# dcmlr/groundgrid

Hardware: AMD Instinct MI355X
Metric: point clouds/s (Velodyne-64, ~120k pts, 120m/0.33m grid) (higher is better)
Workload: dtype f32+f64 (the reference's mixed float/double arithmetic, bit-exact)

## Files before the change

groundgrid_amd/csrc/gg_context.hip:

```cpp
#include <float.h>
#include <math.h>
#include <stdio.h>
#include <string.h>

#include <algorithm>
#include <atomic>
#include <condition_variable>
#include <cstdlib>
#include <cstdio>
#include <functional>
#include <mutex>
#include <string>
#include <thread>
#include <vector>
#include <chrono>

#include <dlfcn.h>
#include <sched.h>
#include <unistd.h>

#include "gg_internal.h"
#include "host_helper.h"
#include "scroll_core.h"
#include "sweep_core.h"
// ... 1045 lines not shown
    g.tiles_c = (n + TILE - 1) / TILE;
    g.T = g.tiles_r * g.tiles_c;
    g.resolution = res;
    g.inv_resolution = 1.0 / res;
    g.length0 = g.length1 = (double)n * res;
    g.half0 = 0.5 * g.length0;
    g.half1 = 0.5 * g.length1;
    g.resolution_f = (float)res;
    g.min_dist_squared = geom.min_dist_squared;
    g.center = n / 2 - 1;
    a.hist_pitch = (g.T + 3) & ~3;
    a.n_slots = n_slots;
    if (g.T > 65535 || (size_t)4 * a.hist_pitch * sizeof(uint32_t) > 150 * 1024) {
        gg_destroy(ctx);
        return GG_ERR_GEOMETRY;
    }
    a.PW = g.T <= 1024 ? (n_slots >= PW_BIG_CONTEXT_SLOTS ? 2048 : 1024) : 8192;
    if (getenv("GG_PW")) a.PW = atoi(getenv("GG_PW"));
    if (a.PW < 64 || a.PW % 64 != 0) {
        gg_destroy(ctx);
        return GG_ERR_INVALID;
    }
    a.tune_sweep_waves = getenv("GG_SWEEP_WAVES") ? atoi(getenv("GG_SWEEP_WAVES")) : 0;
    a.tune_sweep_gpw = getenv("GG_SWEEP_GPW") ? atoi(getenv("GG_SWEEP_GPW")) : 0;
    a.tune_sweep_split = getenv("GG_SWEEP_SPLIT") ? atoi(getenv("GG_SWEEP_SPLIT")) : 0;
    a.tune_sweep_pair = getenv("GG_SWEEP_PAIR") ? atoi(getenv("GG_SWEEP_PAIR")) : 0;
    a.tune_sweep_pair_wgs = getenv("GG_SWEEP_PAIR_WGS") ? atoi(getenv("GG_SWEEP_PAIR_WGS")) : 0;
    a.tune_sweep_pair_waves = getenv("GG_SWEEP_PAIR_WAVES") ? atoi(getenv("GG_SWEEP_PAIR_WAVES")) : 0;
    a.tune_front = getenv("GG_FRONT") ? atoi(getenv("GG_FRONT")) : 0;
    a.tune_k2_per_cloud = getenv("GG_K2_PER_CLOUD") ? atoi(getenv("GG_K2_PER_CLOUD")) : 0;
    a.tune_k2_dense_share = getenv("GG_K2_DENSE_SHARE") ? atoi(getenv("GG_K2_DENSE_SHARE")) : 0;
    a.k2_skip = getenv("GG_K2_SKIP") ? atoi(getenv("GG_K2_SKIP")) : 0;
    a.NCH = (int)((max_points + a.PW - 1) / a.PW);
    make_dev_config(ctx->cfg, a.cfg);

    ctx->h_expected.resize((size_t)g.C);
    for (size_t i = 0; i < cellCount; ++i)
        for (size_t j = 0; j < cellCount; ++j) {
            const float dist = (float)hypot((double)i - (double)cellCount / 2.0, (double)j - (double)cellCount / 2.0);
            ctx->h_expected[i + j * cellCount] = atanf(1 / dist) / geom.vertical_point_ang_dist;
        }

    ctx->sweep_params = gg::sweep::make_params(n, res, geom.min_dist_squared, ctx->cfg.occupied_cells_decrease_factor);
    if (gg::sweep_lds_bytes(ctx->sweep_params) > 158 * 1024) {
        gg_destroy(ctx);
        return GG_ERR_GEOMETRY;
    }
    std::vector<uint16_t> tile_rank(g.T), rank_tile(g.T);
    {
        std::vector<std::pair<uint32_t, int>> order(g.T);
        for (int tc = 0; tc < g.tiles_c; ++tc)
            for (int tr = 0; tr < g.tiles_r; ++tr) order[tr + tc * g.tiles_r] = {morton2((uint32_t)tr, (uint32_t)tc), tr + tc * g.tiles_r};
        std::sort(order.begin(), order.end());
        for (int r = 0; r < g.T; ++r) {
            rank_tile[r] = (uint16_t)order[r].second;
            tile_rank[order[r].second] = (uint16_t)r;
        }
    }

    const size_t A = 256;
    size_t off = 0;
    auto carve = [&](size_t bytes) {
        const size_t o = off;
        off = align_up(off + bytes, A);
        return o;
    };
    const size_t C = (size_t)g.C;
    const size_t Cpad = align_up(C * 4, A) / 4;
    const size_t Npad = align_up(max_points * 8, A) / 8;
    const size_t o_expected = carve(C * 4);
    const size_t o_ptable = carve(C * 16);
    const size_t o_trank = carve((size_t)g.T * 2);
    const size_t o_rtile = carve((size_t)g.T * 2);
    const size_t o_rcell0 = carve((size_t)g.T * 4);
    const size_t percall_slot_floats = align_up((size_t)g.T * PERCALL_BLOCK * 4, A) / 4;
    const size_t o_layers = carve((size_t)n_slots * percall_slot_floats * 4);
    a.gpl = make_gp_layout(n);
    a.gp_bits_off = (int)align_up((size_t)a.gpl.elems, 16);
    a.gp_bits_words = (a.gpl.elems / 64 + 2 + 1) & ~1;
    a.gp2_stride = align_up(((size_t)a.gp_bits_off + (size_t)a.gp_bits_words) * 8, A) / 8;
    a.gp_bits_stride = a.gp2_stride;
    const size_t o_gp2 = carve((size_t)n_slots * a.gp2_stride * 8);
    const size_t o_rec = carve((size_t)n_slots * Npad * 8);
    const size_t o_sorted = carve((size_t)n_slots * Npad * 8);
    a.zcell_stride = align_up((Npad + (size_t)32 * g.T + 64) * 4, A) / 4;
    const size_t o_zcell = carve((size_t)n_slots * a.zcell_stride * 4);
    a.hist_stride = align_up((size_t)a.NCH * a.hist_pitch * 4, A) / 4;
    const size_t o_hist = carve((size_t)n_slots * a.hist_stride * 4);
    a.emit_stride = align_up((size_t)a.NCH * 4 * 4, A) / 4;
    const size_t o_emit = carve((size_t)n_slots * a.emit_stride * 4);
    const size_t o_totals = carve((size_t)n_slots * 4 * 4);
    a.tile_start_stride = align_up((size_t)(g.T + 1) * 4, A) / 4;
    const size_t o_tstart = carve((size_t)n_slots * a.tile_start_stride * 4);
    a.tile_live_stride = align_up((size_t)g.T, A);
    const size_t o_tlive = carve((size_t)n_slots * a.tile_live_stride * 4);
    a.tile_list_stride = align_up((size_t)g.T * 16, A) / 16;
    const size_t o_tlist = carve((size_t)n_slots * a.tile_list_stride * 16);
    const size_t o_tlcnt = carve((size_t)n_slots * 2 * 4);
    const size_t o_fsync = carve(((size_t)2 * n_slots + 16) * 4);
    const size_t o_ssync = carve(64);
    const size_t o_fsync2 = carve(((size_t)2 * n_slots + 16) * 4);
    const size_t o_ssync2 = carve(64);
    const size_t o_scansync = carve((size_t)n_slots * SCAN_SYNC_WORDS * 8);
    const size_t o_scansync2 = carve((size_t)n_slots * SCAN_SYNC_WORDS * 8);
    a.sweep_xchg_stride = align_up(std::max<size_t>(gg::sweep_xchg_entries(ctx->sweep_params), 1) * 16, A) / 8;
    const size_t o_xchg = carve((size_t)n_slots * a.sweep_xchg_stride * 8);
    a.sweep_rec_stride = gg::sweep_pair_rec_floats(ctx->sweep_params);
    a.sweep_rec_clouds = a.sweep_rec_stride ? std::min(n_slots, SWEEP_PAIR_MAX_CLOUDS) : 0;
    const size_t o_srec = carve(std::max<size_t>((size_t)a.sweep_rec_clouds * a.sweep_rec_stride * 4, 64));
    const size_t o_params = carve((size_t)PARAM_RING * n_slots * sizeof(CloudParams));
    const size_t o_gparams = carve(sizeof(CloudParams));
    const size_t o_spts = carve(max_points * sizeof(gg_point16));
    const size_t o_slab = carve(max_points);
    const size_t o_sidx = carve(max_points * 4);
    const size_t o_scnt = carve(64);
    const size_t o_scls = carve(max_points);
    const size_t o_scell = carve(max_points * 4);
    size_t o_apts[GG_ASYNC_DEPTH], o_alab[GG_ASYNC_DEPTH], o_aidx[GG_ASYNC_DEPTH], o_acnt[GG_ASYNC_DEPTH];
    for (int k = 0; k < GG_ASYNC_DEPTH; ++k) {
        o_apts[k] = carve(max_points * sizeof(gg_point16));
        o_acnt[k] = carve(64 + max_points * 5 + 64);
// ... 5 lines not shown
    const size_t gp_valid_words = ((size_t)a.gpl.elems + 31) / 32;
    const size_t o_gpvalid = carve(gp_valid_words * 4);
    std::vector<int> gp_border;
    for (int col = 0; col < n; ++col)
        for (int row = 0; row < n; ++row)
            if (std::max(std::abs(row - a.gpl.c), std::abs(col - a.gpl.c)) >= a.gpl.c) gp_border.push_back(gp_index(a.gpl, row, col));
    a.gp_border_n = (int)gp_border.size();
    const size_t o_gpborder = carve(std::max<size_t>(gp_border.size() * 4, 64));
    a.gp_fresh_cell = 1 + (a.gpl.VS - 1) * 64;
    const size_t o_dbg = carve(64 * 8);
    const size_t o_pdbg = carve(2048 * 8);
    const bool k2_timing = getenv("GG_K2_DEBUG") && (atoi(getenv("GG_K2_DEBUG")) == 9 || atoi(getenv("GG_K2_DEBUG")) == 5 || atoi(getenv("GG_K2_DEBUG")) == 6);
    const size_t o_k2dbg = carve(k2_timing ? (size_t)K2_DBG_WGS * 32 * 8 : 64);
    const size_t o_slotmaps = carve((size_t)n_slots * sizeof(ExportMap));
    ctx->arena_bytes = off;
    CREATE_CHK(hipMalloc(&ctx->d_arena, ctx->arena_bytes));
    char *base = (char *)ctx->d_arena;
    CREATE_CHK(hipMemsetAsync(base, 0, ctx->arena_bytes, ctx->stream));

    a.expected = (const float *)(base + o_expected);
    a.patch_table = (const float4 *)(base + o_ptable);
    a.tile_rank = (const uint16_t *)(base + o_trank);
    a.rank_tile = (const uint16_t *)(base + o_rtile);
    a.rank_cell0 = (const uint32_t *)(base + o_rcell0);
    a.layers = (float *)(base + o_layers);
    a.gp2 = (float2 *)(base + o_gp2);
    a.gp_bits = (unsigned long long *)(base + o_gp2) + a.gp_bits_off;
    a.slot_layer_stride = percall_slot_floats;
    a.rec = (uint2 *)(base + o_rec);
    a.sorted = (uint2 *)(base + o_sorted);
    a.zcell = (float *)(base + o_zcell);
    a.point_stride = Npad;
    a.hist = (uint32_t *)(base + o_hist);
    a.chunk_emit = (uint32_t *)(base + o_emit);
    a.totals = (uint32_t *)(base + o_totals);
    a.tile_start = (uint32_t *)(base + o_tstart);
    a.tile_live = (uint32_t *)(base + o_tlive);
    a.tile_list = (uint4 *)(base + o_tlist);
    a.tile_list_cnt = (uint32_t *)(base + o_tlcnt);
    a.front_sync = (uint32_t *)(base + o_fsync);
    a.sweep_sync = (uint32_t *)(base + o_ssync);
    a.front_sync2 = (uint32_t *)(base + o_fsync2);
    a.sweep_sync2 = (uint32_t *)(base + o_ssync2);
    a.scan_sync = (unsigned long long *)(base + o_scansync);
    a.scan_sync2 = (unsigned long long *)(base + o_scansync2);
    {
        const uint32_t first_epoch[4] = {0u, 0u, 1u, 0u};
        CREATE_CHK(hipMemcpyAsync(a.sweep_sync, first_epoch, sizeof first_epoch, hipMemcpyHostToDevice, ctx->stream));
        const uint32_t first_epoch2[4] = {0u, 0u, 0x80000001u, 0u};
        CREATE_CHK(hipMemcpyAsync(a.sweep_sync2, first_epoch2, sizeof first_epoch2, hipMemcpyHostToDevice, ctx->stream));
        CREATE_CHK(hipStreamSynchronize(ctx->stream));
    }
    {
        CREATE_CHK(hipHostMalloc((void **)&ctx->h_dev_error, 64, hipHostMallocMapped));
        *ctx->h_dev_error = 0u;
        void *dptr = nullptr;
        CREATE_CHK(hipHostGetDevicePointer(&dptr, (void *)ctx->h_dev_error, 0));
        a.dev_error = (uint32_t *)dptr;
    }
    a.sweep_xchg = (unsigned long long *)(base + o_xchg);
    a.sweep_rec = a.sweep_rec_clouds ? (float *)(base + o_srec) : nullptr;
    a.pair_dbg = getenv("GG_PAIR_TIMING") ? (unsigned long long *)(base + o_pdbg) : nullptr;
    a.flags = 0;
    a.k2_debug = getenv("GG_K2_DEBUG") ? atoi(getenv("GG_K2_DEBUG")) : 0;
    a.k2_dbg = (unsigned long long *)(base + o_k2dbg);
    a.k3_debug = getenv("GG_K3_DEBUG") ? atoi(getenv("GG_K3_DEBUG")) : 0;
// ... 1801 lines not shown
    hp[0] = CloudParams{};
    hp[0].slot = slot;
    hp[0].n_points = (int)n;
    hp[0].ox = origin[0], hp[0].oy = origin[1], hp[0].oz = origin[2];
    hp[0].pos_x = ctx->pos_x[slot];
    hp[0].pos_y = ctx->pos_y[slot];
    hp[0].no_confidence = ctx->no_confidence[slot] ? 1 : 0;
    hp[0].fresh = 0;
    HIPCHK(ctx, hipMemcpyAsync(dp, hp, sizeof(CloudParams), hipMemcpyHostToDevice, s));
    BatchIO io{};
    io.d_points = ctx->d_stage_pts;
    io.cloud_stride = ctx->max_points;
    io.point_format = GG_POINT16;
    const int front = launch_classify(a, dp, io, 1, (int)n, s);
    if (front == FRONT_THREE_LAUNCHES) launch_scan(a, dp, 1, s);
    if (front != FRONT_ONE_LAUNCH) launch_scatter(a, dp, 1, (int)n, s);
    launch_stage_insert(a, dp, s);
    launch_fill_bytes((uint8_t *)(a.tile_live + (size_t)slot * a.tile_live_stride), (size_t)a.g.T * 4, 0xFF, s);
    launch_decode_classes(a, slot, n, ctx->d_stage_class, ctx->d_stage_cell, s);
    HIPCHK(ctx, hipGetLastError());
    if (out_class) HIPCHK(ctx, hipMemcpyAsync(out_class, ctx->d_stage_class, n, hipMemcpyDeviceToHost, s));
    if (out_cell) HIPCHK(ctx, hipMemcpyAsync(out_cell, ctx->d_stage_cell, n * 4, hipMemcpyDeviceToHost, s));
    HIPCHK(ctx, ctx->ring.recorded(r, s));
    ctx->lazy_pending[slot] = 0;
    if (const int rc = own_stream_mutated_map(ctx)) return rc;
    SYNCCHK(ctx, hipStreamSynchronize(s));
    return GG_OK;
}

extern "C" int gg_debug_set_tuning(gg_context *ctx, const char *key, int value)
{
    if (!ctx || !key || value < 0) return GG_ERR_INVALID;
    if (!strcmp(key, "pw")) return ctx->arena.PW;
    if (!strcmp(key, "graph_replays")) return (int)std::min<long>(ctx->graph_replays, 1 << 30);
    if (!strcmp(key, "fresh_count")) {
        int c = 0;
        for (int k = 0; k < ctx->n_slots; ++k) c += ctx->fresh[k] ? 1 : 0;
        return c;
    }
    if (!strcmp(key, "lazy_count")) {
        int c = 0;
        for (int k = 0; k < ctx->n_slots; ++k) c += ctx->lazy_pending[k] ? 1 : 0;
        return c;
    }
    if (!strcmp(key, "export_variant_default")) return EXPORT_VARIANT_DEFAULT;
    if (!strcmp(key, "import_variant_default")) return IMPORT_VARIANT_DEFAULT;
    if (!strcmp(key, "images_variant_default")) return IMAGES_VARIANT_DEFAULT;
    if (!strcmp(key, "graphs")) {
        ctx->graphs_enabled = value != 0;
        drop_graphs(ctx);
        return GG_OK;
    }
    drop_graphs(ctx);
    if (!strcmp(key, "sweep_waves")) ctx->arena.tune_sweep_waves = value;
    else if (!strcmp(key, "sweep_gpw")) ctx->arena.tune_sweep_gpw = value;
    else if (!strcmp(key, "sweep_split")) ctx->arena.tune_sweep_split = value;
    else if (!strcmp(key, "sweep_pair")) ctx->arena.tune_sweep_pair = value;
    else if (!strcmp(key, "sweep_pair_wgs")) ctx->arena.tune_sweep_pair_wgs = value;
    else if (!strcmp(key, "sweep_pair_waves")) ctx->arena.tune_sweep_pair_waves = value;
    else if (!strcmp(key, "fresh_maps")) ctx->fresh_enabled = value != 0;
    else if (!strcmp(key, "front")) ctx->arena.tune_front = std::min(value, 3);
    else if (!strcmp(key, "sweep_poll_cap")) ctx->arena.tune_sweep_poll_cap = value;
    else if (!strcmp(key, "scan_parts")) ctx->arena.tune_scan_parts = value;
    else if (!strcmp(key, "scan_poll_cap")) ctx->arena.tune_scan_poll_cap = value;
    else if (!strcmp(key, "upload_pieces")) ctx->upload_pieces = value;
    else if (!strcmp(key, "results_direct")) ctx->results_direct = value;
// ... 85 lines not shown
```

groundgrid_amd/csrc/gg_internal.h:

```cpp
#pragma once

#include <hip/hip_runtime.h>
#include <stdint.h>

#include <atomic>
#include <mutex>

#include "groundgrid_hip.h"
#include "gp_layout.h"

namespace gg {

constexpr int TILE = 16;
constexpr int TILE_CELLS = TILE * TILE;
constexpr uint32_t KEY_OUTSIDE = 0xFFFFFFFFu;
constexpr int K2_DBG_WGS = 32768;
constexpr int PW_BIG_CONTEXT_SLOTS = 128;
constexpr int SWEEP_LATENCY_MAX_CLOUDS = 256;
constexpr int K2_MIN_GROUPS_PER_CLOUD = 64;
constexpr int PACKED_TILE_COUNTERS_MIN_T = 1024;
constexpr int K2_LIGHT_MAX = 512;
constexpr int KEY_TILE_SHIFT = 12;
constexpr int SCAN_MAX_PARTS = 16, SCAN_SYNC_WORDS = 1 + SCAN_MAX_PARTS;
constexpr uint32_t KEY_EMIT_BIT = 1u << 10;
// ... 36 lines not shown
    int slot;
    int n_points;
    float ox, oy, oz;
    float base_z;
    double pos_x, pos_y;
    int has_tf;
    int fresh;
    int no_confidence;
    double tf[12];
    int label_shift;
    int io_index;
    int cfg_index = -1;
};

struct Arena {
    Geometry g;
    DevConfig cfg;
    const float *expected;
    const float4 *patch_table;
    const uint16_t *tile_rank;
    const uint16_t *rank_tile;
    const uint32_t *rank_cell0;
    float *layers;  size_t slot_layer_stride;
    const uint32_t *gp_valid;
    float2 *gp2;    size_t gp2_stride;    GpLayout gpl;
    unsigned long long *gp_bits;  size_t gp_bits_stride;  int gp_fresh_cell;
    int gp_bits_off, gp_bits_words;
    const int *gp_border;  int gp_border_n;
    int fresh_launch;
    uint2 *rec;     uint2 *sorted;  size_t point_stride;
    float *zcell;   size_t zcell_stride;
    uint32_t *hist;        size_t hist_stride;
    int hist_pitch;
    uint32_t *front_sync;
    uint32_t *dev_error;
    uint32_t *chunk_emit;  size_t emit_stride;
    uint32_t *totals;
    uint32_t *tile_start;  size_t tile_start_stride;
    uint32_t *tile_live;   size_t tile_live_stride;
    uint4 *tile_list;      size_t tile_list_stride;
    uint32_t *tile_list_cnt;
    unsigned long long *scan_sync;
    uint32_t *front_sync2, *sweep_sync2;
    unsigned long long *scan_sync2;
    uint32_t *sweep_sync;
    unsigned long long *sweep_xchg; size_t sweep_xchg_stride;
    float *sweep_rec; size_t sweep_rec_stride; int sweep_rec_clouds;
    unsigned long long *pair_dbg;
    int n_slots;
    int PW;
    int NCH;
    int tune_sweep_waves;
    int tune_sweep_gpw;
    int tune_sweep_split;
    int tune_sweep_pair;
    int tune_sweep_pair_wgs;
    int tune_sweep_pair_waves;
    int tune_sweep_poll_cap;
    int tune_sweep_fault;
    int tune_scan_fault;
    int tune_scan_poll_cap;
    int tune_scan_parts;
    int tune_front;
    int tune_k2_per_cloud;
    int tune_k2_dense_share;
    int k2_skip;
// ... 251 lines not shown
```

groundgrid_amd/csrc/k1_classify.hip:

```cpp
#include "gg_device.h"
#include "sort_core.h"

#include <algorithm>

namespace gg {

constexpr int WALK_MAX_STEP = 1 << 16;
constexpr int WALK_PACKED_MAX = 12;

struct PointIn {
    float x, y, z;
    int ring;
};

template <int FMT>
GG_DEV PointIn load_point(const void *base, size_t idx)
{
    PointIn p;
    if (FMT == GG_POINT16) {
        const uint4 v = reinterpret_cast<const uint4 *>(base)[idx];
        p.x = __uint_as_float(v.x);
        p.y = __uint_as_float(v.y);
        p.z = __uint_as_float(v.z);
        p.ring = (int)(v.w & 0xFFFFu);
// ... 175 lines not shown
                const uint32_t x = (home + k) % nc, size = q + (x < r ? 1u : 0u);
                const uint32_t t = __hip_atomic_fetch_add(&tickets[x], 1u, __ATOMIC_RELAXED, __HIP_MEMORY_SCOPE_AGENT);
                if (t < size) got = x * q + (x < r ? x : r) + t;
            }
            s_word = got;
        }
        __syncthreads();
        item = s_word;
        if (item == 0xFFFFFFFFu) return;
    } else {
        item = xcd_contiguous_item(blockIdx.x + blockIdx.y * gridDim.x, n_items);
    }
    const int cloud = (int)(item / gridDim.x), bx = (int)(item % gridDim.x);
    const CloudParams &cp = params[cloud];
    DevConfig own_cfg;
    if (SC) load_cloud_config(a, cp.cfg_index, own_cfg);
    const DevConfig &cfg = SC ? own_cfg : a.cfg;
    const int chunk = bx * 4 + wave;
    const int n = cp.n_points;
    const int nch = (n + a.PW - 1) / a.PW;
    const int groups_of_cloud = max(1, (nch + 3) / 4);
    if (bx >= groups_of_cloud) return;
    for (int t = threadIdx.x; t < T; t += 256) lds_tile_rank[t] = a.tile_rank[t];
    uint32_t *hist = lds_hist + wave * words;
    for (int t = lane; t < words; t += 64) hist[t] = 0u;
    __syncthreads();
    const bool active = chunk < nch;

    const float2 *gp2 = gp2_ptr(a, cp.slot);
    const char *pts = reinterpret_cast<const char *>(io.d_points) +
                      (size_t)cp.io_index * io.cloud_stride * (FMT == GG_POINT16 ? 16 : 32);
    uint2 *rec = a.rec + (size_t)cp.slot * a.point_stride;
    const __amdgpu_buffer_rsrc_t ghist = words_rsrc(a.hist + (size_t)cp.slot * a.hist_stride, a.hist_stride);
    const uint32_t row = (uint32_t)chunk * (uint32_t)TP;

    const int base = chunk * a.PW;
    const int end = min(base + a.PW, n);
    if (active) {
        uint32_t n_kept = 0, n_ign = 0, n_outl = 0, n_inmap = 0;
        constexpr int ITEMS = 4;
        PointIn pt[ITEMS];
#pragma unroll
        for (int j = 0; j < ITEMS; ++j) pt[j] = load_point<FMT>(pts, (size_t)min(base + j * 64 + lane, end - 1));
        for (int p0 = base; p0 < end; p0 += 64 * ITEMS) {
            PointIn pt_next[ITEMS];
#pragma unroll
            for (int j = 0; j < ITEMS; ++j) pt_next[j] = load_point<FMT>(pts, (size_t)min(p0 + 64 * ITEMS + j * 64 + lane, end - 1));
            bool valid[ITEMS];
#pragma unroll
            for (int j = 0; j < ITEMS; ++j) valid[j] = p0 + j * 64 + lane < end;
            if (cp.has_tf) {
#pragma unroll
                for (int j = 0; j < ITEMS; ++j) transform_point(cp.tf, pt[j].x, pt[j].y, pt[j].z);
            }
            int gi0[ITEMS], gi1[ITEMS];
            bool inmap_[ITEMS];
            float og[ITEMS];
#pragma unroll
            for (int j = 0; j < ITEMS; ++j) inmap_[j] = locate_point(a, cp, pt[j], gi0[j], gi1[j]) && valid[j];
            const bool need_ground = !cp.no_confidence;
#pragma unroll
            for (int j = 0; j < ITEMS; ++j) og[j] = gp2[(inmap_[j] && need_ground) ? gp_idx(a, gi0[j], gi1[j]) : 0].x;
#pragma unroll
            for (int j = 0; j < ITEMS; ++j) {
                const int p = p0 + j * 64 + lane;
                int cls = GG_CLASS_KEPT;
                bool walk = false;
                if (inmap_[j]) cls = classify_point(a, cfg, cp, pt[j], og[j], walk);
                const int n_walk = __popcll(__ballot(walk));
                if (n_walk > WALK_PACKED_MAX) {
                    if (walk && ray_walk_hits_lane(a, cfg, cp, gp2, pt[j].x, pt[j].y, pt[j].z)) cls = GG_CLASS_OUTLIER;
                } else if (n_walk > 0) {
                    const unsigned long long hits = walk_packed(a, cfg, cp, gp2, pt[j].x, pt[j].y, pt[j].z, walk, lane);
                    if ((hits >> lane) & 1ull) cls = GG_CLASS_OUTLIER;
                }
                uint32_t key = KEY_OUTSIDE;
                if (inmap_[j]) key = make_key(a, lds_tile_rank, gi0[j], gi1[j], cls);
                if (valid[j]) rec[p] = make_uint2(__float_as_uint(pt[j].z), key);
                const bool inmap = key != KEY_OUTSIDE;
                const uint32_t tr = key >> KEY_TILE_SHIFT;
                const LaneRun run = lane_run(inmap ? tr : 0x100000u, lane);
                if (inmap && run.head) {
                    const uint32_t len = (uint32_t)__popcll(run.mask);
                    if (packed)
                        atomicAdd(&hist[tr >> 1], len << ((tr & 1u) * 16u));
                    else
                        atomicAdd(&hist[tr], len);
                }
                const bool emit = inmap && (key & KEY_EMIT_BIT);
                n_inmap += (uint32_t)__popcll(__ballot(inmap));
                n_kept += (uint32_t)__popcll(__ballot(emit && cls == GG_CLASS_KEPT));
                n_ign += (uint32_t)__popcll(__ballot(emit && cls == GG_CLASS_IGNORED));
                n_outl += (uint32_t)__popcll(__ballot(inmap && cls == GG_CLASS_OUTLIER));
            }
#pragma unroll
            for (int j = 0; j < ITEMS; ++j) pt[j] = pt_next[j];
        }

        for (int g = lane; g < TP / 4; g += 64) {
            u32x4 v;
#pragma unroll
            for (int k = 0; k < 4; ++k) {
                const int t = 4 * g + k;
                v[k] = packed ? (hist[t >> 1] >> ((t & 1) * 16)) & 0xFFFFu : hist[t];
            }
            store16_row<SHAPE != FRONT_THREE_LAUNCHES>(ghist, row + 4u * (uint32_t)g, v);
        }
        if (lane == 0) {
            const u32x4 v = {n_kept, n_ign, n_outl, n_inmap};
            store16_row<SHAPE != FRONT_THREE_LAUNCHES>(words_rsrc(a.chunk_emit + (size_t)cp.slot * a.emit_stride, a.emit_stride), 4u * (uint32_t)chunk, v);
        }
    }
    if (SHAPE == FRONT_THREE_LAUNCHES) return;

    drain_vector_memory();
    __syncthreads();
    uint32_t *arrivals = a.front_sync + (size_t)cp.slot, *scanned = a.front_sync + (size_t)a.n_slots + (size_t)cp.slot;
    if (threadIdx.x == 0) s_word = __hip_atomic_fetch_add(arrivals, 1u, __ATOMIC_RELAXED, __HIP_MEMORY_SCOPE_AGENT);
    __syncthreads();
    const bool last = s_word == (uint32_t)groups_of_cloud - 1u;
    if (last) {
        scan_cloud<4, true>(a, cp, nch, s_scan);
        if (SHAPE == FRONT_ONE_LAUNCH) {
            drain_vector_memory();
            __syncthreads();
            if (threadIdx.x == 0) __hip_atomic_store(scanned, 1u, __ATOMIC_RELAXED, __HIP_MEMORY_SCOPE_AGENT);
        }
    }
    if (SHAPE != FRONT_ONE_LAUNCH) return;

    if (!last) {
        __syncthreads();
        if (threadIdx.x == 0) {
            uint32_t polls = 0;
            while (__hip_atomic_load(scanned, __ATOMIC_RELAXED, __HIP_MEMORY_SCOPE_AGENT) == 0u && polls < FRONT_WAIT_POLLS) {
                __builtin_amdgcn_s_sleep(16);
                ++polls;
            }
            s_word = polls < FRONT_WAIT_POLLS ? 1u : 0u;
            if (polls >= FRONT_WAIT_POLLS) __hip_atomic_store(a.dev_error, (uint32_t)GG_DEVERR_FRONT_WAIT, __ATOMIC_RELAXED, __HIP_MEMORY_SCOPE_SYSTEM);
        }
        __syncthreads();
        if (s_word == 0u) return;
    }
    if (!active) return;
    uint2 *sorted = a.sorted + (size_t)cp.slot * a.point_stride;
    if (packed) {
        for (int t = lane; t < words; t += 64) hist[t] = 0u;
        scatter_chunk<true, true>(hist, ghist, row, rec, sorted, base, end, lane);
    } else {
        for (int g = lane; g < TP / 4; g += 64) *reinterpret_cast<u32x4 *>(hist + 4 * g) = load16_agent(ghist, row + 4u * (uint32_t)g);
        scatter_chunk<false, true>(hist, ghist, row, rec, sorted, base, end, lane);
    }
}

size_t classify_lds_bytes(const Arena &a)
{
    const bool packed = a.g.T > PACKED_TILE_COUNTERS_MIN_T && a.PW < 65536;
    return (size_t)4 * (packed ? a.hist_pitch / 2 : a.hist_pitch) * sizeof(uint32_t) + (((size_t)a.g.T * 2 + 15) & ~(size_t)15) + 64;
}

template <int FMT, int SHAPE>
static void launch_classify_as(const Arena &a, const CloudParams *d_params, const BatchIO &io, dim3 grid, size_t lds, int n_counters, hipStream_t s)
{
    if (a.slot_cfg_launch) hipLaunchKernelGGL((k_classify<FMT, SHAPE, true>), grid, dim3(256), lds, s, a, d_params, io, n_counters);
    else hipLaunchKernelGGL((k_classify<FMT, SHAPE>), grid, dim3(256), lds, s, a, d_params, io, n_counters);
}

static int front_resident_groups(size_t lds, bool sc)
{
    int dev = 0, cus = 0, per_cu = 0;
    if (hipGetDevice(&dev) != hipSuccess) return 0;
    if (hipDeviceGetAttribute(&cus, hipDeviceAttributeMultiprocessorCount, dev) != hipSuccess) return 0;
    if (hipOccupancyMaxActiveBlocksPerMultiprocessor(&per_cu, sc ? reinterpret_cast<const void *>(k_classify<GG_POINT16, FRONT_ONE_LAUNCH, true>) : reinterpret_cast<const void *>(k_classify<GG_POINT16, FRONT_ONE_LAUNCH>), 256, lds) != hipSuccess) return 0;
    return std::max(0, per_cu - 1) * cus;
}

int launch_classify(const Arena &a, const CloudParams *d_params, const BatchIO &io, int n_clouds, int max_n, hipStream_t s)
{
    const int nch = (max_n + a.PW - 1) / a.PW;
    if (n_clouds == 0) return FRONT_ONE_LAUNCH;
    const int groups = std::max(1, (nch + 3) / 4);
// ... 178 lines not shown
```

groundgrid_amd/csrc/k_sort.hip:

```cpp
#include "gg_device.h"
#include "sort_core.h"

#include <algorithm>

namespace gg {

__global__ __launch_bounds__(1024) void k_scan(const Arena a, const CloudParams *__restrict__ params)
{
    __shared__ uint32_t lds[32];
    __shared__ u32x4 part[1024];
    const CloudParams cp = params[blockIdx.x];
    scan_cloud<16, false>(a, cp, (cp.n_points + a.PW - 1) / a.PW, lds, part);
}

__global__ __launch_bounds__(1024) void k_scan_parts(const Arena a, const CloudParams *__restrict__ params)
{
    __shared__ uint32_t lds[32];
    __shared__ u32x4 part[1024];
    const CloudParams cp = params[blockIdx.y];
    unsigned long long *sync = a.scan_sync + (size_t)blockIdx.y * SCAN_SYNC_WORDS;
    if (threadIdx.x == 0) lds[0] = __hip_atomic_fetch_add(reinterpret_cast<uint32_t *>(sync), 1u, __ATOMIC_RELAXED, __HIP_MEMORY_SCOPE_AGENT);
    __syncthreads();
    const int my_part = (int)lds[0];
    __syncthreads();
    scan_cloud<16, false>(a, cp, (cp.n_points + a.PW - 1) / a.PW, lds, part, my_part, (int)gridDim.x, sync + 1);
}

int scan_parts(const Arena &a, int n_clouds)
{
    const int G = a.hist_pitch / 4;
    if (a.tune_scan_parts > 0) return std::max((G + SCAN_PART_MAX_GROUPS - 1) / SCAN_PART_MAX_GROUPS, std::min(a.tune_scan_parts, SCAN_MAX_PARTS));
    if (G < 512 || n_clouds >= 512) return 1;
    return std::max((G + SCAN_PART_MAX_GROUPS - 1) / SCAN_PART_MAX_GROUPS, std::min(std::min(SCAN_MAX_PARTS, G / 64), 512 / n_clouds));
}

void launch_scan(const Arena &a, const CloudParams *d_params, int n_clouds, hipStream_t s)
{
    if (n_clouds == 0) return;
    const int parts = scan_parts(a, n_clouds);
    if (parts <= 1) {
        hipLaunchKernelGGL(k_scan, dim3(n_clouds), dim3(1024), 0, s, a, d_params);
        return;
    }
    hipMemsetAsync(a.scan_sync, 0, (size_t)n_clouds * SCAN_SYNC_WORDS * sizeof(unsigned long long), s);
    hipLaunchKernelGGL(k_scan_parts, dim3(parts, n_clouds), dim3(1024), 0, s, a, d_params);
}

__global__ __launch_bounds__(256) void k_scatter(const Arena a, const CloudParams *__restrict__ params)
{
    extern __shared__ __attribute__((aligned(16))) uint32_t lds_offs[];
    const uint32_t item = xcd_contiguous_item(blockIdx.x + blockIdx.y * gridDim.x, gridDim.x * gridDim.y);
    const int cloud = (int)(item / gridDim.x), bx = (int)(item % gridDim.x);
    const CloudParams cp = params[cloud];
    const int wave = threadIdx.x >> 6, lane = threadIdx.x & 63;
    const int chunk = bx * 4 + wave;
    const int n = cp.n_points;
    const int nch = (n + a.PW - 1) / a.PW;
    if (chunk >= nch) return;

    const int T = a.g.T, TP = a.hist_pitch;
    const bool packed = T > PACKED_TILE_COUNTERS_MIN_T && a.PW < 65536;
    const int words = packed ? TP / 2 : TP;
    uint32_t *offs = lds_offs + wave * words;
    const __amdgpu_buffer_rsrc_t ghist = words_rsrc(a.hist + (size_t)cp.slot * a.hist_stride, a.hist_stride);
    const uint32_t row = (uint32_t)chunk * (uint32_t)TP;
    const uint2 *rec = a.rec + (size_t)cp.slot * a.point_stride;
    uint2 *sorted = a.sorted + (size_t)cp.slot * a.point_stride;
    const int base = chunk * a.PW;
    const int end = min(base + a.PW, n);
    if (packed) {
        for (int t = lane; t < words; t += 64) offs[t] = 0u;
        scatter_chunk<true, false>(offs, ghist, row, rec, sorted, base, end, lane);
    } else {
        for (int g = lane; g < TP / 4; g += 64) *reinterpret_cast<u32x4 *>(offs + 4 * g) = load16_row<false>(ghist, row + 4u * (uint32_t)g);
        scatter_chunk<false, false>(offs, ghist, row, rec, sorted, base, end, lane);
    }
}

void launch_scatter(const Arena &a, const CloudParams *d_params, int n_clouds, int max_n, hipStream_t s)
{
    const int nch = (max_n + a.PW - 1) / a.PW;
    if (nch == 0 || n_clouds == 0) return;
    dim3 grid((nch + 3) / 4, n_clouds);
    const bool packed = a.g.T > PACKED_TILE_COUNTERS_MIN_T && a.PW < 65536;
    const size_t lds = (size_t)4 * (packed ? a.hist_pitch / 2 : a.hist_pitch) * sizeof(uint32_t);
    static PerDeviceOnce big_lds;
    if (lds > 64 * 1024)
        big_lds.run([] { hipFuncSetAttribute(reinterpret_cast<const void *>(k_scatter), hipFuncAttributeMaxDynamicSharedMemorySize, 160 * 1024); });
    hipLaunchKernelGGL(k_scatter, grid, dim3(256), lds, s, a, d_params);
}

}
```

groundgrid_amd/csrc/sort_core.h:

```cpp
#pragma once

#include "gg_device.h"

namespace gg {

typedef uint32_t u32x4 __attribute__((ext_vector_type(4)));

constexpr int AUX_SC1 = 16;

GG_DEV __amdgpu_buffer_rsrc_t words_rsrc(const uint32_t *base, size_t words)
{
    return __builtin_amdgcn_make_buffer_rsrc(const_cast<uint32_t *>(base), 0, (int)(words * 4), 0x00020000);
}
GG_DEV u32x4 load16_agent(__amdgpu_buffer_rsrc_t r, uint32_t word) { return __builtin_amdgcn_raw_buffer_load_b128(r, word * 4u, 0, AUX_SC1); }
GG_DEV void store16_agent(__amdgpu_buffer_rsrc_t r, uint32_t word, u32x4 v) { __builtin_amdgcn_raw_buffer_store_b128(v, r, word * 4u, 0, AUX_SC1); }
GG_DEV void drain_vector_memory() { __asm__ volatile("s_waitcnt vmcnt(0)" ::: "memory"); }

GG_DEV uint32_t wave_inclusive_scan(uint32_t v, int lane)
{
#pragma unroll
    for (int d = 1; d < 64; d <<= 1) {
        const uint32_t o = __shfl_up(v, d, 64);
        if (lane >= d) v += o;
    }
    return v;
}

template <int NW>
GG_DEV uint32_t block_exclusive_scan(uint32_t v, uint32_t *lds , uint32_t &total)
{
    const int lane = threadIdx.x & 63, wave = threadIdx.x >> 6;
    const uint32_t inc = wave_inclusive_scan(v, lane);
    __syncthreads();
    if (lane == 63) lds[wave] = inc;
    __syncthreads();
    if (wave == 0) {
        const uint32_t w = (lane < NW) ? lds[lane] : 0u;
        const uint32_t winc = wave_inclusive_scan(w, lane);
        if (lane < NW) lds[lane] = winc - w;
        if (lane == NW - 1) lds[NW] = winc;
    }
    __syncthreads();
    total = lds[NW];
    return lds[wave] + inc - v;
}

template <bool AGENT> GG_DEV u32x4 load16_row(__amdgpu_buffer_rsrc_t r, uint32_t word)
{
    return AGENT ? load16_agent(r, word) : __builtin_amdgcn_raw_buffer_load_b128(r, word * 4u, 0, 0);
}
template <bool AGENT> GG_DEV void store16_row(__amdgpu_buffer_rsrc_t r, uint32_t word, u32x4 v)
{
    if (AGENT) store16_agent(r, word, v);
    else __builtin_amdgcn_raw_buffer_store_b128(v, r, word * 4u, 0, 0);
}

constexpr uint32_t SCAN_WAIT_POLLS = 1u << 24;
constexpr int SCAN_PART_MAX_GROUPS = 1024;
static_assert(4 * SCAN_PART_MAX_GROUPS < (1 << 15), "the light / dense tile counts of a scan part must fit their 15-bit fields");
template <int NW, bool AGENT>
GG_DEV void scan_cloud(const Arena &a, const CloudParams &cp, int nch, uint32_t *lds , u32x4 *part = nullptr ,
                       int my_part = 0, int n_parts = 1, unsigned long long *sync = nullptr )
{
    constexpr int NT = 64 * NW;
    const int tid = threadIdx.x;
    const int T = a.g.T, TP = a.hist_pitch, G = TP / 4;
    const __amdgpu_buffer_rsrc_t hist = words_rsrc(a.hist + (size_t)cp.slot * a.hist_stride, a.hist_stride);
    uint32_t *tile_start = a.tile_start + (size_t)cp.slot * a.tile_start_stride;
    uint32_t *tile_live = a.tile_live + (size_t)cp.slot * a.tile_live_stride;
    uint4 *tile_list = a.tile_list + (size_t)cp.slot * a.tile_list_stride;
    const int Gp = (G + n_parts - 1) / n_parts;
    const int G_lo = min(G, my_part * Gp), G_hi = min(G, G_lo + Gp);
    const int GS = part ? min(NT, (max(G_hi - G_lo, 1) + 63) & ~63) : NT, Q = part ? NT / GS : 1;
    const int gi = tid % GS, q = tid / GS;
    const int c_lo = q < Q ? (int)((long long)nch * q / Q) : 0, c_hi = q < Q ? (int)((long long)nch * (q + 1) / Q) : 0;

    uint32_t carry = 0, lcarry = 0, dcarry = 0;
    for (int g0 = G_lo; g0 < G_hi || (sync && g0 == G_lo); g0 += GS) {
        const int g = g0 + gi;
        const bool have = g < G_hi && q < Q;
        u32x4 s = {0u, 0u, 0u, 0u};
        if (have) {
#pragma unroll 16
            for (int c = c_lo; c < c_hi; ++c) s += load16_row<AGENT>(hist, (uint32_t)c * (uint32_t)TP + 4u * (uint32_t)g);
        }
        u32x4 before = {0u, 0u, 0u, 0u};
        if (part && Q > 1) {
            __syncthreads();
            part[tid] = s;
            __syncthreads();
            u32x4 all = {0u, 0u, 0u, 0u};
            for (int k = 0; k < Q; ++k) {
                const u32x4 v = part[k * GS + gi];
                if (k < q) before += v;
                all += v;
            }
            s = all;
        }
        const bool lead = have && q == 0;
        uint32_t total;
        const uint32_t excl_lead = block_exclusive_scan<NW>(lead ? s.x + s.y + s.z + s.w : 0u, lds, total);
        uint32_t excl = excl_lead;
        if (part && Q > 1) {
            __syncthreads();
            if (lead) part[gi].x = excl_lead;
            __syncthreads();
            excl = part[gi].x;
        }
        {
            uint32_t nl = 0, nd = 0;
#pragma unroll
            for (int k = 0; k < 4; ++k) {
                const bool in = lead && 4 * g + k < T;
                nd += (in && s[k] > (uint32_t)K2_LIGHT_MAX) ? 1u : 0u;
                nl += (in && s[k] > 0u && s[k] <= (uint32_t)K2_LIGHT_MAX) ? 1u : 0u;
// ... 8 lines not shown
                if (tid < my_part) {
                    uint32_t polls = 0;
                    const uint32_t poll_cap = a.tune_scan_poll_cap > 0 ? (uint32_t)a.tune_scan_poll_cap : SCAN_WAIT_POLLS;
                    while (((w = __hip_atomic_load(&sync[tid], __ATOMIC_RELAXED, __HIP_MEMORY_SCOPE_AGENT)) >> 63) == 0ull && polls < poll_cap) {
                        __builtin_amdgcn_s_sleep(16);
                        ++polls;
                    }
                    if ((w >> 63) == 0ull) __hip_atomic_store(a.dev_error, (uint32_t)GG_DEVERR_SCAN_WAIT, __ATOMIC_RELAXED, __HIP_MEMORY_SCOPE_SYSTEM);
                }
                const bool mine = tid < my_part;
                uint32_t before_t, before_l;
                block_exclusive_scan<NW>(mine ? (uint32_t)w : 0u, lds, before_t);
                block_exclusive_scan<NW>(mine ? (uint32_t)((w >> 32) & 0x7FFFu) | ((uint32_t)((w >> 47) & 0x7FFFu) << 16) : 0u, lds, before_l);
                carry = before_t;
                lcarry = before_l & 0xFFFFu;
                dcarry = before_l >> 16;
            }
            uint32_t li = lcarry + (lexcl & 0xFFFFu), di = dcarry + (lexcl >> 16), start = carry + excl;
#pragma unroll
            for (int k = 0; k < 4; ++k) {
                const int t = 4 * g + k;
                if (lead && t < T) {
                    const uint4 entry = make_uint4((uint32_t)t, start, start + s[k], a.rank_cell0[t]);
                    if (s[k] == 0u) tile_live[t] = 0u;
                    else if (s[k] > (uint32_t)K2_LIGHT_MAX) tile_list[(uint32_t)T - 1u - di++] = entry;
                    else tile_list[li++] = entry;
                    tile_start[t] = start;
                    start += s[k];
                }
            }
            lcarry += ltotal & 0xFFFFu;
            dcarry += ltotal >> 16;
        }
        if (have) {
            u32x4 run;
            run.x = carry + excl;
            run.y = run.x + s.x;
            run.z = run.y + s.y;
            run.w = run.z + s.z;
            run += before;
#pragma unroll 16
            for (int c = c_lo; c < c_hi; ++c) {
                const uint32_t w = (uint32_t)c * (uint32_t)TP + 4u * (uint32_t)g;
                const u32x4 h = load16_row<AGENT>(hist, w);
                store16_row<AGENT>(hist, w, run);
                run += h;
            }
        }
        carry += total;
    }
    if (tid == 0 && my_part == n_parts - 1) {
        tile_start[T] = carry;
        uint32_t *lc = a.tile_list_cnt + (size_t)cp.slot * 2;
        lc[0] = lcarry;
        lc[1] = dcarry;
    }
    if (my_part != 0) return;

    const __amdgpu_buffer_rsrc_t ce = words_rsrc(a.chunk_emit + (size_t)cp.slot * a.emit_stride, a.emit_stride);
    uint32_t *ce_out = a.chunk_emit + (size_t)cp.slot * a.emit_stride;
    u32x4 kcarry = {0u, 0u, 0u, 0u};
    for (int c0 = 0; c0 < nch; c0 += NT) {
        const int c = c0 + tid;
        u32x4 v = {0u, 0u, 0u, 0u}, e;
        if (c < nch) v = load16_row<AGENT>(ce, 4u * (uint32_t)c);
#pragma unroll
        for (int k = 0; k < 4; ++k) {
            uint32_t total;
            e[k] = kcarry[k] + block_exclusive_scan<NW>(v[k], lds, total);
            kcarry[k] += total;
        }
        if (c < nch) *reinterpret_cast<u32x4 *>(ce_out + 4 * (size_t)c) = e;
    }
    if (tid == 0) *reinterpret_cast<u32x4 *>(a.totals + (size_t)cp.slot * 4) = kcarry;
}

template <bool PACKED, bool AGENT>
GG_DEV void scatter_chunk(uint32_t *offs, __amdgpu_buffer_rsrc_t hist, uint32_t row_word, const uint2 *__restrict__ rec, uint2 *__restrict__ sorted,
                          int base, int end, int lane)
// ... 62 lines not shown
```

Measured before the change: 223,600.

## Group per-chunk tile histograms into four-chunk rows with packed 16-bit prefixes

```diff
diff --git a/groundgrid_amd/csrc/gg_context.hip b/groundgrid_amd/csrc/gg_context.hip
--- a/groundgrid_amd/csrc/gg_context.hip
+++ b/groundgrid_amd/csrc/gg_context.hip
@@ -1101,6 +1101,16 @@
     a.tune_k2_dense_share = getenv("GG_K2_DENSE_SHARE") ? atoi(getenv("GG_K2_DENSE_SHARE")) : 0;
     a.k2_skip = getenv("GG_K2_SKIP") ? atoi(getenv("GG_K2_SKIP")) : 0;
     a.NCH = (int)((max_points + a.PW - 1) / a.PW);
+    a.front_rows = (g.T <= PACKED_TILE_COUNTERS_MIN_T && (long long)3 * a.PW < 65536) ? 1 : 4;
+    if (const char *e = getenv("GG_FRONT_ROWS")) {
+        const int v = atoi(e);
+        if (v != 1 && v != 4) {
+            gg_destroy(ctx);
+            return GG_ERR_INVALID;
+        }
+        if (v == 4) a.front_rows = 4;
+    }
+    a.hist_pre_pitch = (g.T + 7) & ~7;
     make_dev_config(ctx->cfg, a.cfg);
 
     ctx->h_expected.resize((size_t)g.C);
@@ -1154,8 +1164,11 @@
     const size_t o_sorted = carve((size_t)n_slots * Npad * 8);
     a.zcell_stride = align_up((Npad + (size_t)32 * g.T + 64) * 4, A) / 4;
     const size_t o_zcell = carve((size_t)n_slots * a.zcell_stride * 4);
-    a.hist_stride = align_up((size_t)a.NCH * a.hist_pitch * 4, A) / 4;
+    const size_t hist_groups = ((size_t)a.NCH + 3) / 4;
+    a.hist_stride = align_up((a.front_rows == 1 ? hist_groups : (size_t)a.NCH) * a.hist_pitch * 4, A) / 4;
     const size_t o_hist = carve((size_t)n_slots * a.hist_stride * 4);
+    a.hist_pre_stride = a.front_rows == 1 ? align_up(hist_groups * 3 * a.hist_pre_pitch * 2, A) / 2 : 0;
+    const size_t o_hpre = carve(std::max<size_t>((size_t)n_slots * a.hist_pre_stride * 2, 64));
     a.emit_stride = align_up((size_t)a.NCH * 4 * 4, A) / 4;
     const size_t o_emit = carve((size_t)n_slots * a.emit_stride * 4);
     const size_t o_totals = carve((size_t)n_slots * 4 * 4);
@@ -1227,6 +1240,7 @@
     a.zcell = (float *)(base + o_zcell);
     a.point_stride = Npad;
     a.hist = (uint32_t *)(base + o_hist);
+    a.hist_pre = (uint16_t *)(base + o_hpre);
     a.chunk_emit = (uint32_t *)(base + o_emit);
     a.totals = (uint32_t *)(base + o_totals);
     a.tile_start = (uint32_t *)(base + o_tstart);
@@ -3094,6 +3108,7 @@
 {
     if (!ctx || !key || value < 0) return GG_ERR_INVALID;
     if (!strcmp(key, "pw")) return ctx->arena.PW;
+    if (!strcmp(key, "front_rows")) return ctx->arena.front_rows;
     if (!strcmp(key, "graph_replays")) return (int)std::min<long>(ctx->graph_replays, 1 << 30);
     if (!strcmp(key, "fresh_count")) {
         int c = 0;
diff --git a/groundgrid_amd/csrc/gg_internal.h b/groundgrid_amd/csrc/gg_internal.h
--- a/groundgrid_amd/csrc/gg_internal.h
+++ b/groundgrid_amd/csrc/gg_internal.h
@@ -92,6 +92,9 @@
     float *zcell;   size_t zcell_stride;
     uint32_t *hist;        size_t hist_stride;
     int hist_pitch;
+    uint16_t *hist_pre;    size_t hist_pre_stride;
+    int hist_pre_pitch;
+    int front_rows;
     uint32_t *front_sync;
     uint32_t *dev_error;
     uint32_t *chunk_emit;  size_t emit_stride;
diff --git a/groundgrid_amd/csrc/k1_classify.hip b/groundgrid_amd/csrc/k1_classify.hip
--- a/groundgrid_amd/csrc/k1_classify.hip
+++ b/groundgrid_amd/csrc/k1_classify.hip
@@ -231,6 +231,7 @@
                       (size_t)cp.io_index * io.cloud_stride * (FMT == GG_POINT16 ? 16 : 32);
     uint2 *rec = a.rec + (size_t)cp.slot * a.point_stride;
     const __amdgpu_buffer_rsrc_t ghist = words_rsrc(a.hist + (size_t)cp.slot * a.hist_stride, a.hist_stride);
+    const bool grouped = a.front_rows == 1;
     const uint32_t row = (uint32_t)chunk * (uint32_t)TP;
 
     const int base = chunk * a.PW;
@@ -296,18 +297,44 @@
             for (int j = 0; j < ITEMS; ++j) pt[j] = pt_next[j];
         }
 
-        for (int g = lane; g < TP / 4; g += 64) {
+        int wave_again = wave;
+        __asm__ volatile("" : "+v"(wave_again));
+        const int chunk_again = bx * 4 + wave_again;
+        const uint32_t row_again = (uint32_t)chunk_again * (uint32_t)TP;
+        const uint32_t *hrow = lds_hist + wave_again * words;
+        for (int g = lane; g < TP / 4 && !grouped; g += 64) {
             u32x4 v;
 #pragma unroll
             for (int k = 0; k < 4; ++k) {
                 const int t = 4 * g + k;
-                v[k] = packed ? (hist[t >> 1] >> ((t & 1) * 16)) & 0xFFFFu : hist[t];
-            }
-            store16_row<SHAPE != FRONT_THREE_LAUNCHES>(ghist, row + 4u * (uint32_t)g, v);
+                v[k] = packed ? (hrow[t >> 1] >> ((t & 1) * 16)) & 0xFFFFu : hrow[t];
+            }
+            store16_row<SHAPE != FRONT_THREE_LAUNCHES>(ghist, row_again + 4u * (uint32_t)g, v);
         }
         if (lane == 0) {
             const u32x4 v = {n_kept, n_ign, n_outl, n_inmap};
-            store16_row<SHAPE != FRONT_THREE_LAUNCHES>(words_rsrc(a.chunk_emit + (size_t)cp.slot * a.emit_stride, a.emit_stride), 4u * (uint32_t)chunk, v);
+            store16_row<SHAPE != FRONT_THREE_LAUNCHES>(words_rsrc(a.chunk_emit + (size_t)cp.slot * a.emit_stride, a.emit_stride), 4u * (uint32_t)chunk_again, v);
+        }
+    }
+    if (grouped) {
+        __syncthreads();
+        if (bx * 4 < nch) {
+            const __amdgpu_buffer_rsrc_t gpre = pre_rsrc(a, cp.slot);
+            for (int g = lane + 64 * wave; 8 * g < TP; g += 256) {
+                const bool second = 8 * g + 4 < TP;
+                u32x4 lo = {0u, 0u, 0u, 0u}, hi = {0u, 0u, 0u, 0u};
+#pragma unroll
+                for (int w = 0; w < 4; ++w) {
+                    if (w > 0 && bx * 4 + w < nch) {
+                        const u32x4 p = {lo.x | (lo.y << 16), lo.z | (lo.w << 16), hi.x | (hi.y << 16), hi.z | (hi.w << 16)};
+                        store16_row<SHAPE != FRONT_THREE_LAUNCHES>(gpre, pre_row_word(a, bx, w) + 4u * (uint32_t)g, p);
+                    }
+                    lo += *reinterpret_cast<const u32x4 *>(lds_hist + w * words + 8 * g);
+                    if (second) hi += *reinterpret_cast<const u32x4 *>(lds_hist + w * words + 8 * g + 4);
+                }
+                store16_row<SHAPE != FRONT_THREE_LAUNCHES>(ghist, (uint32_t)bx * (uint32_t)TP + 8u * (uint32_t)g, lo);
+                if (second) store16_row<SHAPE != FRONT_THREE_LAUNCHES>(ghist, (uint32_t)bx * (uint32_t)TP + 8u * (uint32_t)g + 4u, hi);
+            }
         }
     }
     if (SHAPE == FRONT_THREE_LAUNCHES) return;
@@ -319,7 +346,7 @@
     __syncthreads();
     const bool last = s_word == (uint32_t)groups_of_cloud - 1u;
     if (last) {
-        scan_cloud<4, true>(a, cp, nch, s_scan);
+        scan_cloud<4, true, 4>(a, cp, nch, hist_rows(a, nch), s_scan);
         if (SHAPE == FRONT_ONE_LAUNCH) {
             drain_vector_memory();
             __syncthreads();
@@ -347,6 +374,9 @@
     if (packed) {
         for (int t = lane; t < words; t += 64) hist[t] = 0u;
         scatter_chunk<true, true>(hist, ghist, row, rec, sorted, base, end, lane);
+    } else if (grouped) {
+        load_group_offsets<true>(a, hist, ghist, pre_rsrc(a, cp.slot), bx, wave, lane);
+        scatter_chunk<false, true>(hist, ghist, row, rec, sorted, base, end, lane);
     } else {
         for (int g = lane; g < TP / 4; g += 64) *reinterpret_cast<u32x4 *>(hist + 4 * g) = load16_agent(ghist, row + 4u * (uint32_t)g);
         scatter_chunk<false, true>(hist, ghist, row, rec, sorted, base, end, lane);
diff --git a/groundgrid_amd/csrc/k_sort.hip b/groundgrid_amd/csrc/k_sort.hip
--- a/groundgrid_amd/csrc/k_sort.hip
+++ b/groundgrid_amd/csrc/k_sort.hip
@@ -10,7 +10,8 @@
     __shared__ uint32_t lds[32];
     __shared__ u32x4 part[1024];
     const CloudParams cp = params[blockIdx.x];
-    scan_cloud<16, false>(a, cp, (cp.n_points + a.PW - 1) / a.PW, lds, part);
+    const int nch = (cp.n_points + a.PW - 1) / a.PW;
+    scan_cloud<16, false, 8>(a, cp, nch, hist_rows(a, nch), lds, part);
 }
 
 __global__ __launch_bounds__(1024) void k_scan_parts(const Arena a, const CloudParams *__restrict__ params)
@@ -23,7 +24,8 @@
     __syncthreads();
     const int my_part = (int)lds[0];
     __syncthreads();
-    scan_cloud<16, false>(a, cp, (cp.n_points + a.PW - 1) / a.PW, lds, part, my_part, (int)gridDim.x, sync + 1);
+    const int nch = (cp.n_points + a.PW - 1) / a.PW;
+    scan_cloud<16, false, 8>(a, cp, nch, hist_rows(a, nch), lds, part, my_part, (int)gridDim.x, sync + 1);
 }
 
 int scan_parts(const Arena &a, int n_clouds)
@@ -71,6 +73,9 @@
     if (packed) {
         for (int t = lane; t < words; t += 64) offs[t] = 0u;
         scatter_chunk<true, false>(offs, ghist, row, rec, sorted, base, end, lane);
+    } else if (a.front_rows == 1) {
+        load_group_offsets<false>(a, offs, ghist, pre_rsrc(a, cp.slot), bx, wave, lane);
+        scatter_chunk<false, false>(offs, ghist, row, rec, sorted, base, end, lane);
     } else {
         for (int g = lane; g < TP / 4; g += 64) *reinterpret_cast<u32x4 *>(offs + 4 * g) = load16_row<false>(ghist, row + 4u * (uint32_t)g);
         scatter_chunk<false, false>(offs, ghist, row, rec, sorted, base, end, lane);
diff --git a/groundgrid_amd/csrc/sort_core.h b/groundgrid_amd/csrc/sort_core.h
--- a/groundgrid_amd/csrc/sort_core.h
+++ b/groundgrid_amd/csrc/sort_core.h
@@ -54,12 +54,47 @@
     if (AGENT) store16_agent(r, word, v);
     else __builtin_amdgcn_raw_buffer_store_b128(v, r, word * 4u, 0, 0);
 }
+constexpr uint32_t ROW_NO_ACCESS = 0x80000000u;
+template <bool AGENT> GG_DEV u32x4 load16_row_if(__amdgpu_buffer_rsrc_t r, uint32_t word, bool on)
+{
+    return __builtin_amdgcn_raw_buffer_load_b128(r, on ? word * 4u : ROW_NO_ACCESS, 0, AGENT ? AUX_SC1 : 0);
+}
+template <bool AGENT> GG_DEV void store16_row_if(__amdgpu_buffer_rsrc_t r, uint32_t word, u32x4 v, bool on)
+{
+    __builtin_amdgcn_raw_buffer_store_b128(v, r, on ? word * 4u : ROW_NO_ACCESS, 0, AGENT ? AUX_SC1 : 0);
+}
+
+GG_DEV int hist_rows(const Arena &a, int nch) { return a.front_rows == 1 ? (nch + 3) / 4 : nch; }
+GG_DEV __amdgpu_buffer_rsrc_t pre_rsrc(const Arena &a, int slot)
+{
+    return words_rsrc(reinterpret_cast<const uint32_t *>(a.hist_pre + (size_t)slot * a.hist_pre_stride), a.hist_pre_stride / 2);
+}
+GG_DEV uint32_t pre_row_word(const Arena &a, int gr, int w) { return ((uint32_t)gr * 3u + (uint32_t)(w - 1)) * (uint32_t)(a.hist_pre_pitch / 2); }
+
+template <bool AGENT>
+GG_DEV void load_group_offsets(const Arena &a, uint32_t *offs, __amdgpu_buffer_rsrc_t hist, __amdgpu_buffer_rsrc_t pre, int gr, int w, int lane)
+{
+    const int TP = a.hist_pitch;
+    const uint32_t row = (uint32_t)gr * (uint32_t)TP, prow = pre_row_word(a, gr, max(w, 1));
+    for (int g = lane; 8 * g < TP; g += 64) {
+        const bool second = 8 * g + 4 < TP;
+        u32x4 lo = load16_row<AGENT>(hist, row + 8u * (uint32_t)g);
+        u32x4 hi = load16_row_if<AGENT>(hist, row + 8u * (uint32_t)g + 4u, second);
+        if (w > 0) {
+            const u32x4 p = load16_row<AGENT>(pre, prow + 4u * (uint32_t)g);
+            lo += u32x4{p.x & 0xFFFFu, p.x >> 16, p.y & 0xFFFFu, p.y >> 16};
+            hi += u32x4{p.z & 0xFFFFu, p.z >> 16, p.w & 0xFFFFu, p.w >> 16};
+        }
+        *reinterpret_cast<u32x4 *>(offs + 8 * g) = lo;
+        if (second) *reinterpret_cast<u32x4 *>(offs + 8 * g + 4) = hi;
+    }
+}
 
 constexpr uint32_t SCAN_WAIT_POLLS = 1u << 24;
 constexpr int SCAN_PART_MAX_GROUPS = 1024;
 static_assert(4 * SCAN_PART_MAX_GROUPS < (1 << 15), "the light / dense tile counts of a scan part must fit their 15-bit fields");
-template <int NW, bool AGENT>
-GG_DEV void scan_cloud(const Arena &a, const CloudParams &cp, int nch, uint32_t *lds , u32x4 *part = nullptr ,
+template <int NW, bool AGENT, int KEEP>
+GG_DEV void scan_cloud(const Arena &a, const CloudParams &cp, int nch, int nrows, uint32_t *lds , u32x4 *part = nullptr ,
                        int my_part = 0, int n_parts = 1, unsigned long long *sync = nullptr )
 {
     constexpr int NT = 64 * NW;
@@ -73,14 +108,21 @@
     const int G_lo = min(G, my_part * Gp), G_hi = min(G, G_lo + Gp);
     const int GS = part ? min(NT, (max(G_hi - G_lo, 1) + 63) & ~63) : NT, Q = part ? NT / GS : 1;
     const int gi = tid % GS, q = tid / GS;
-    const int c_lo = q < Q ? (int)((long long)nch * q / Q) : 0, c_hi = q < Q ? (int)((long long)nch * (q + 1) / Q) : 0;
+    const int c_lo = q < Q ? (int)((long long)nrows * q / Q) : 0, c_hi = q < Q ? (int)((long long)nrows * (q + 1) / Q) : 0;
+    const bool keep = (nrows + Q - 1) / Q <= KEEP;
 
     uint32_t carry = 0, lcarry = 0, dcarry = 0;
     for (int g0 = G_lo; g0 < G_hi || (sync && g0 == G_lo); g0 += GS) {
         const int g = g0 + gi;
         const bool have = g < G_hi && q < Q;
         u32x4 s = {0u, 0u, 0u, 0u};
-        if (have) {
+        u32x4 h[KEEP];
+        if (keep) {
+#pragma unroll
+            for (int k = 0; k < KEEP; ++k) h[k] = load16_row_if<AGENT>(hist, (uint32_t)(c_lo + k) * (uint32_t)TP + 4u * (uint32_t)g, have && c_lo + k < c_hi);
+#pragma unroll
+            for (int k = 0; k < KEEP; ++k) s += h[k];
+        } else if (have) {
 #pragma unroll 16
             for (int c = c_lo; c < c_hi; ++c) s += load16_row<AGENT>(hist, (uint32_t)c * (uint32_t)TP + 4u * (uint32_t)g);
         }
@@ -155,19 +197,27 @@
             lcarry += ltotal & 0xFFFFu;
             dcarry += ltotal >> 16;
         }
-        if (have) {
+        {
             u32x4 run;
             run.x = carry + excl;
             run.y = run.x + s.x;
             run.z = run.y + s.y;
             run.w = run.z + s.z;
             run += before;
+            if (keep) {
+#pragma unroll
+                for (int k = 0; k < KEEP; ++k) {
+                    store16_row_if<AGENT>(hist, (uint32_t)(c_lo + k) * (uint32_t)TP + 4u * (uint32_t)g, run, have && c_lo + k < c_hi);
+                    run += h[k];
+                }
+            } else if (have) {
 #pragma unroll 16
-            for (int c = c_lo; c < c_hi; ++c) {
-                const uint32_t w = (uint32_t)c * (uint32_t)TP + 4u * (uint32_t)g;
-                const u32x4 h = load16_row<AGENT>(hist, w);
-                store16_row<AGENT>(hist, w, run);
-                run += h;
+                for (int c = c_lo; c < c_hi; ++c) {
+                    const uint32_t w = (uint32_t)c * (uint32_t)TP + 4u * (uint32_t)g;
+                    const u32x4 hc = load16_row<AGENT>(hist, w);
+                    store16_row<AGENT>(hist, w, run);
+                    run += hc;
+                }
             }
         }
         carry += total;
```

New measurement: 226,700 (median of 6 runs). 1.4% higher.
